# wangxb29/PPST

Measured on AMD Instinct MI355X. Metric: 512x512 portrait swaps/sec/GPU, higher is better.
Workload: dtype bf16x3 (fp32 split into hi+lo bf16, 3 MFMA passes, fp32 accumulate); 1 GPU; simple_swapping 512x512 batch=8 per GPU, generator+encoders forward only (BASELINE configs[1]); image_parallel=1 batch per rank, no data-path collective

## Files before the change

ppst_amd/csrc/conv1x1.hip:

```cpp
#include "common.h"

struct C1Args {
  const float* x;
  const unsigned char* wpack;
  const int4* steps;
  float* y;
  const float* bias;
  const float* noise;
  const float* prelu;
  float* stats;
  const float* residual;
  float noise_weight, out_scale;
  int B, hw, in_ld, out_ld, cout, nsteps, act, res_ld, n_tiles, tiles;
  int in_h, in_w, out_h, out_w, tiles_x, pad_mode;
  const float* in_ss;
  const float* in_prelu;
  int in_c, in_act;
  const float* in_res;
  int in_res_ld;
};

#define C1_GROUP 8
#define C1_BLOB 8192

typedef _Float16 __attribute__((ext_vector_type(8))) c1_half8;
template <int PREC>
__device__ __forceinline__ void c1_cvt(float v, unsigned short& h, unsigned short& l) {
  if (PREC == 0) split_bf16(v, h, l);
  else if (PREC == 3) { h = __builtin_bit_cast(unsigned short, (_Float16)v); l = 0; }
  else { h = f2bf(v); l = 0; }
}
template <int PREC>
__device__ __forceinline__ void c1_cvt8(const float (&v)[8], bf16x8& hi, bf16x8& lo) {
  if (PREC == 3) {
#pragma unroll
    for (int j = 0; j < 8; ++j) {
      unsigned short h, l;
      c1_cvt<PREC>(v[j], h, l);
      hi[j] = (short)h;
      lo[j] = (short)l;
    }
    return;
  }
  uint2 h0, l0 = make_uint2(0u, 0u), h1, l1 = make_uint2(0u, 0u);
  if (PREC == 0) {
    split_bf16x4(make_float4(v[0], v[1], v[2], v[3]), h0, l0);
    split_bf16x4(make_float4(v[4], v[5], v[6], v[7]), h1, l1);
  } else {
    h0 = f2bf_x4(make_float4(v[0], v[1], v[2], v[3]));
    h1 = f2bf_x4(make_float4(v[4], v[5], v[6], v[7]));
  }
  hi = __builtin_bit_cast(bf16x8, make_uint4(h0.x, h0.y, h1.x, h1.y));
  lo = __builtin_bit_cast(bf16x8, make_uint4(l0.x, l0.y, l1.x, l1.y));
}
template <int IOS>
__device__ __forceinline__ void c1_unpack8(float4 r, float (&v)[8]) {
  const float4 a = st_unpack4<IOS>(make_uint2(__float_as_uint(r.x), __float_as_uint(r.y)));
  const float4 b = st_unpack4<IOS>(make_uint2(__float_as_uint(r.z), __float_as_uint(r.w)));
  v[0] = a.x; v[1] = a.y; v[2] = a.z; v[3] = a.w; v[4] = b.x; v[5] = b.y; v[6] = b.z; v[7] = b.w;
}
template <int PREC>
__device__ __forceinline__ f32x4 c1_mfma(bf16x8 bh, bf16x8 bl, bf16x8 xh, bf16x8 xl, f32x4 acc) {
  if (PREC == 0) {
    acc = __builtin_amdgcn_mfma_f32_16x16x32_bf16(bh, xl, acc, 0, 0, 0);
    acc = __builtin_amdgcn_mfma_f32_16x16x32_bf16(bl, xh, acc, 0, 0, 0);
    return __builtin_amdgcn_mfma_f32_16x16x32_bf16(bh, xh, acc, 0, 0, 0);
  }
  if (PREC == 3) return __builtin_amdgcn_mfma_f32_16x16x32_f16(__builtin_bit_cast(c1_half8, bh), __builtin_bit_cast(c1_half8, xh), acc, 0, 0, 0);
  return __builtin_amdgcn_mfma_f32_16x16x32_bf16(bh, xh, acc, 0, 0, 0);
}

__device__ __forceinline__ int c1_pad(int i, int n, int mode) {
  if (mode == PPST_PAD_REFLECT) {
    if (i < 0) i = -i;
    if (i >= n) i = 2 * (n - 1) - i;
  }
  return i < 0 ? 0 : (i >= n ? n - 1 : i);
}

template <int MT, int NT, bool TAPS, bool SPEC = true, int IOS = PPST_ST_F32>
__device__ __forceinline__ void c1_epilogue(const C1Args& a, f32x4 (&acc)[MT][NT], float (&red)[8][NT > 4 ? 128 : 64][2], int b, int mblk,
                                            int ntile, int pbase, int oy0, int ox, int tid, int wave, int r16, int g) {
  const int act = a.act & 0xff;
  const bool res_after = (a.act >> 8) & 1;
  const float slope = (act == PPST_ACT_PRELU && a.prelu) ? a.prelu[0] : 0.f;
  float4 s1[NT], s2[NT];
#pragma unroll
  for (int nt = 0; nt < NT; ++nt) { s1[nt] = make_float4(0.f, 0.f, 0.f, 0.f); s2[nt] = s1[nt]; }
  const int64_t img = (int64_t)b * (TAPS ? a.out_h * a.out_w : a.hw);
  constexpr int ES = IOS == PPST_ST_F32 ? 4 : 2;
  unsigned char* const yb = (unsigned char*)a.y + img * a.out_ld * ES;
  const float* const nzb = a.noise ? a.noise + img : nullptr;
  const unsigned char* const rb = a.residual ? (const unsigned char*)a.residual + img * a.res_ld * ES : nullptr;
  const int nbase = ntile * (NT > 4 ? 128 : 64) + g * 4;
  float nzv[MT];
  float4 bva[NT];
  const __amdgpu_buffer_rsrc_t nrs = __builtin_amdgcn_make_buffer_rsrc((void*)(nzb ? (const void*)nzb : (const void*)yb), 0,
                                                                       nzb ? (TAPS ? a.out_h * a.out_w : a.hw) * 4 : 0, 0x00020000);
#pragma unroll
  for (int mt = 0; mt < MT; ++mt) {
    const int p = pbase + mt * 16 + r16;
    const bool ok = TAPS ? (oy0 + mt < a.out_h && ox < a.out_w) : p < a.hw;
    nzv[mt] = a.noise_weight * __builtin_bit_cast(float, __builtin_amdgcn_raw_buffer_load_b32(
                                   nrs, ok ? (TAPS ? (oy0 + mt) * a.out_w + ox : p) * 4 : (int)0x80000000, 0, 0));
  }
#pragma unroll
  for (int nt = 0; nt < NT; ++nt)
    bva[nt] = __builtin_bit_cast(float4, __builtin_amdgcn_raw_buffer_load_b128(__builtin_amdgcn_make_buffer_rsrc((void*)(a.bias ? (const void*)a.bias : (const void*)a.y), 0, a.bias ? a.cout * 4 : 0, 0x00020000), (nbase + nt * 16) * 4, 0, 0));
  auto epi_passes = [&](auto act_c, auto res_c) {
#pragma clang fp contract(off)
    const int ACT = act_c.value, RES = res_c.value;
#pragma unroll
  for (int mt = 0; mt < MT; ++mt) {
    const int p = pbase + mt * 16 + r16;
    if (TAPS ? (oy0 + mt >= a.out_h || ox >= a.out_w) : p >= a.hw) continue;
    const int pin = TAPS ? (oy0 + mt) * a.out_w + ox : p;
    const int yo = pin * a.out_ld, ro = pin * a.res_ld;
    const float nz = nzv[mt];
#pragma unroll
    for (int nt = 0; nt < NT; ++nt) {
      const int n0 = nbase + nt * 16;
      if (n0 >= a.cout) continue;
      float4 rv = make_float4(0.f, 0.f, 0.f, 0.f);
      const float4 bv = bva[nt];
      if (RES) rv = st_ld4<IOS>(rb, ro + n0);
      float o[4] = {acc[mt][nt][0] + bv.x + nz, acc[mt][nt][1] + bv.y + nz, acc[mt][nt][2] + bv.z + nz, acc[mt][nt][3] + bv.w + nz};
      const float r4[4] = {rv.x, rv.y, rv.z, rv.w};
#pragma unroll
      for (int c = 0; c < 4; ++c) {
        float t = o[c];
        if (RES == 1) t += r4[c];
        if (ACT == PPST_ACT_LRELU) t = (t > 0.f ? t : t * 0.2f) * 1.41421356237309515f;
        else if (ACT == PPST_ACT_PRELU) t = t >= 0.f ? t : t * slope;
        if (RES == 2) t += r4[c];
        o[c] = t * a.out_scale;
      }
      st_st4<IOS>(yb, yo + n0, make_float4(o[0], o[1], o[2], o[3]));
      s1[nt].x += o[0]; s1[nt].y += o[1]; s1[nt].z += o[2]; s1[nt].w += o[3];
      s2[nt].x += o[0] * o[0]; s2[nt].y += o[1] * o[1]; s2[nt].z += o[2] * o[2]; s2[nt].w += o[3] * o[3];
    }
  }
  };
  {
    const int resm = a.residual ? (res_after ? 2 : 1) : 0;
#define EPI_GO(A_)                                                                                    \
  do {                                                                                                \
    if (resm == 0) epi_passes(EpiC<A_>{}, EpiC<0>{});                                                 \
    else if (resm == 1) epi_passes(EpiC<A_>{}, EpiC<1>{});                                            \
    else epi_passes(EpiC<A_>{}, EpiC<2>{});                                                           \
  } while (0)
    if (!SPEC) epi_passes(EpiR{act}, EpiR{resm});
    else if (act == PPST_ACT_LRELU) EPI_GO(PPST_ACT_LRELU);
    else if (act == PPST_ACT_PRELU) EPI_GO(PPST_ACT_PRELU);
    else EPI_GO(PPST_ACT_NONE);
#undef EPI_GO
  }
  if (a.stats) {
#pragma unroll
    for (int nt = 0; nt < NT; ++nt) {
      float4 u = s1[nt], w = s2[nt];
      float* uv[8] = {&u.x, &u.y, &u.z, &u.w, &w.x, &w.y, &w.z, &w.w};
#pragma unroll
      for (int q = 0; q < 8; ++q) {
        float t = *uv[q];
        t += __builtin_bit_cast(float, __builtin_amdgcn_mov_dpp(__builtin_bit_cast(int, t), 0xB1, 0xf, 0xf, true));
        t += __builtin_bit_cast(float, __builtin_amdgcn_mov_dpp(__builtin_bit_cast(int, t), 0x4E, 0xf, 0xf, true));
        t += __builtin_bit_cast(float, __builtin_amdgcn_mov_dpp(__builtin_bit_cast(int, t), 0x141, 0xf, 0xf, true));
        t += __builtin_bit_cast(float, __builtin_amdgcn_mov_dpp(__builtin_bit_cast(int, t), 0x140, 0xf, 0xf, true));
        *uv[q] = t;
      }
      if (r16 == 0) {
        float* r = &red[wave][nt * 16 + g * 4][0];
        r[0] = u.x; r[1] = w.x; r[2] = u.y; r[3] = w.y; r[4] = u.z; r[5] = w.z; r[6] = u.w; r[7] = w.w;
      }
    }
    __syncthreads();
    if (tid < (NT > 4 ? 128 : 64)) {
      const int n = ntile * (NT > 4 ? 128 : 64) + tid;
      if (n < a.cout) {
        float t0 = 0.f, t1 = 0.f;
#pragma unroll
        for (int wv = 0; wv < 8; ++wv) { t0 += red[wv][tid][0]; t1 += red[wv][tid][1]; }
        float* o = a.stats + (((int64_t)b * a.tiles + mblk) * a.cout + n) * 2;
        o[0] = t0;
        o[1] = t1;
      }
    }
  }
}

template <int INSS, bool TAPS = false, int NT_ = 4, int PREC = 0, int IOS = PPST_ST_F32>
__global__ __launch_bounds__(512, 4) void conv1x1_stream_kernel(C1Args a) {
  constexpr int MT = 2, NT = NT_;
  constexpr bool X3 = PREC == 0;
  static_assert(IOS == PPST_ST_F32 || IOS == (PREC == 3 ? PPST_ST_F16 : PREC == 1 ? PPST_ST_BF16 : -1), "half storage: single-pass modes");
  constexpr int ES = IOS == PPST_ST_F32 ? 4 : 2;
  constexpr int BLOB1 = X3 ? C1_BLOB : C1_BLOB / 2;
  __shared__ uint4 sB[C1_GROUP * BLOB1 / 16];
  __shared__ float red[8][64][2];

  const int nwg = gridDim.x;
  int wid;
  {
    int id = blockIdx.x, q = nwg >> 3, r = nwg & 7, xcd = id & 7;
    wid = (xcd < r ? xcd * (q + 1) : r * (q + 1) + (xcd - r) * q) + (id >> 3);
  }
  const int ntile = wid % a.n_tiles;
  int mblk = wid / a.n_tiles;
  const int b = mblk / a.tiles;
  mblk -= b * a.tiles;
  const int tid = threadIdx.x, lane = tid & 63, wave = __builtin_amdgcn_readfirstlane(tid >> 6);
  const int r16 = lane & 15, g = lane >> 4;
  const int pbase = mblk * 256 + wave * 32;
  const int tyi = TAPS ? mblk / a.tiles_x : 0, txi = TAPS ? mblk - tyi * a.tiles_x : 0;
  const int oy0 = tyi * 16 + wave * 2, ox = txi * 16 + r16;
  const unsigned char* xb = (const unsigned char*)a.x + (int64_t)b * (TAPS ? a.in_h * a.in_w : a.hw) * a.in_ld * ES;
  const unsigned char* wblob = a.wpack + (int64_t)ntile * a.nsteps * BLOB1;
#if defined(__HIP_DEVICE_COMPILE__)
  typedef const __attribute__((address_space(4))) int4* StepPtr;
#else
  typedef const int4* StepPtr;
#endif
  StepPtr steps = (StepPtr)a.steps;

  int64_t aoff[MT];
  bool pok[MT];
#pragma unroll
  for (int mt = 0; mt < MT; ++mt) {
    const int p = pbase + mt * 16 + r16;
    pok[mt] = TAPS ? true : p < a.hw;
    aoff[mt] = TAPS ? 0 : (int64_t)(pok[mt] ? p : 0) * a.in_ld + g * 8;
  }
  const float in_slope = (INSS && a.in_act == PPST_ACT_PRELU && a.in_prelu) ? a.in_prelu[0] : 0.f;
  auto in_act = [&](float t) -> float {
    if (a.in_act == PPST_ACT_LRELU) return (t > 0.f ? t : t * 0.2f) * 1.41421356237309515f;
    if (a.in_act == PPST_ACT_PRELU) return t >= 0.f ? t : t * in_slope;
    return t;
  };

  f32x4 acc[MT][NT];
#pragma unroll
  for (int i = 0; i < MT; ++i)
#pragma unroll
    for (int j = 0; j < NT; ++j) acc[i][j] = (f32x4){0.f, 0.f, 0.f, 0.f};

  float4 raw[MT][2], ss[4];
  float4 rres[INSS == 2 ? MT : 1][2];
  auto a_load = [&](int4 d) {
    const int chan = d.x;
    if (TAPS) {
      int ix = ox + d.z;
      bool xok = ix >= 0 && ix < a.in_w;
      ix = c1_pad(ix, a.in_w, a.pad_mode);
#pragma unroll
      for (int mt = 0; mt < MT; ++mt) {
        int iy = oy0 + mt + d.y;
        const bool yok = iy >= 0 && iy < a.in_h;
        iy = c1_pad(iy, a.in_h, a.pad_mode);
        pok[mt] = a.pad_mode != PPST_PAD_ZERO || (xok && yok);
        aoff[mt] = ((int64_t)iy * a.in_w + ix) * a.in_ld + g * 8;
      }
    }
#pragma unroll
    for (int mt = 0; mt < MT; ++mt) {
      const float4* p = (const float4*)(xb + (aoff[mt] + chan) * ES);
      raw[mt][0] = p[0];
      if (IOS == PPST_ST_F32) raw[mt][1] = p[1];
      if (INSS == 2) {
        const int pp = pbase + mt * 16 + r16;
        const float4* q = (const float4*)(a.in_res + ((int64_t)b * a.hw + (pok[mt] ? pp : 0)) * a.in_res_ld + g * 8 + chan);
        rres[mt][0] = q[0];
        rres[mt][1] = q[1];
      }
    }
    if (INSS) {
      const float4* q = (const float4*)(a.in_ss + ((int64_t)b * a.in_c + chan + g * 8) * 2);
      ss[0] = q[0]; ss[1] = q[1]; ss[2] = q[2]; ss[3] = q[3];
    }
  };
  a_load(steps[0]);

  for (int s0 = 0; s0 < a.nsteps; s0 += C1_GROUP) {
    const int ng = a.nsteps - s0 < C1_GROUP ? a.nsteps - s0 : C1_GROUP;
    if (s0) __syncthreads();
    for (int i = tid; i < ng * (BLOB1 / 16); i += 512) sB[i] = ((const uint4*)(wblob + (int64_t)s0 * BLOB1))[i];
    __syncthreads();
    for (int sl = 0; sl < ng; ++sl) {
      const int s = s0 + sl;
      bf16x8 ah[MT], al[MT];
      bool vok[MT];
#pragma unroll
      for (int mt = 0; mt < MT; ++mt) vok[mt] = pok[mt];
#pragma unroll
      for (int mt = 0; mt < MT; ++mt) {
        if (IOS != PPST_ST_F32 && !INSS) {
          const float4 z = vok[mt] ? raw[mt][0] : make_float4(0.f, 0.f, 0.f, 0.f);
          ah[mt] = __builtin_bit_cast(bf16x8, z);
          al[mt] = ah[mt];
          continue;
        }
        float v[8] = {raw[mt][0].x, raw[mt][0].y, raw[mt][0].z, raw[mt][0].w, raw[mt][1].x, raw[mt][1].y, raw[mt][1].z, raw[mt][1].w};
        if (IOS != PPST_ST_F32) c1_unpack8<IOS>(raw[mt][0], v);
        if (INSS) {
          const float sc[8] = {ss[0].x, ss[0].z, ss[1].x, ss[1].z, ss[2].x, ss[2].z, ss[3].x, ss[3].z};
          const float sh[8] = {ss[0].y, ss[0].w, ss[1].y, ss[1].w, ss[2].y, ss[2].w, ss[3].y, ss[3].w};
#pragma unroll
          for (int j = 0; j < 8; ++j) {
            float t = sc[j] * v[j] + sh[j];
            if (INSS == 2) {
              const float4 r4 = rres[mt][j >> 2];
              t += (j & 3) == 0 ? r4.x : (j & 3) == 1 ? r4.y : (j & 3) == 2 ? r4.z : r4.w;
            }
            v[j] = in_act(t);
          }
        }
#pragma unroll
        for (int j = 0; j < 8; ++j)
          if (!vok[mt]) v[j] = 0.f;
        c1_cvt8<PREC>(v, ah[mt], al[mt]);
      }
      if (s + 1 < a.nsteps) a_load(steps[s + 1]);
      const unsigned char* bs = (const unsigned char*)sB + sl * BLOB1 + g * 1024 + r16 * 16;
#pragma unroll
      for (int nt = 0; nt < NT; ++nt) {
        const bf16x8 bh = *(const bf16x8*)(bs + nt * 256);
        bf16x8 bl = bh;
        if (X3) bl = *(const bf16x8*)(bs + nt * 256 + 4096);
#pragma unroll
        for (int mt = 0; mt < MT; ++mt) acc[mt][nt] = c1_mfma<PREC>(bh, bl, ah[mt], al[mt], acc[mt][nt]);
      }
    }
  }

  c1_epilogue<MT, NT, TAPS, X3, IOS>(a, acc, red, b, mblk, ntile, pbase, oy0, ox, tid, wave, r16, g);
}

#define C3_GROUP 9
template <int CTRL>
__device__ __forceinline__ bf16x8 c3_shift(bf16x8 edge, bf16x8 centre) {
  typedef int __attribute__((ext_vector_type(4))) i4;
  const i4 e = __builtin_bit_cast(i4, edge), c = __builtin_bit_cast(i4, centre);
  i4 r;
#pragma unroll
  for (int i = 0; i < 4; ++i) r[i] = __builtin_amdgcn_update_dpp(e[i], c[i], CTRL, 0xf, 0xf, false);
  return __builtin_bit_cast(bf16x8, r);
}

template <bool INSS, int NT_, int PREC = 0, int IOS = PPST_ST_F32>
__global__ __launch_bounds__(512, NT_ > 4 ? 2 : 4) void conv3x3_direct_kernel(C1Args a) {
  constexpr int MT = 2, NT = NT_;
  constexpr bool X3 = PREC == 0;
  static_assert(IOS == PPST_ST_F32 || IOS == (PREC == 3 ? PPST_ST_F16 : PREC == 1 ? PPST_ST_BF16 : -1), "half storage: single-pass modes");
  constexpr int ES = IOS == PPST_ST_F32 ? 4 : 2;
  constexpr int PSTR = (NT > 4 ? 128 : 64) * 16;
  constexpr int BLOB = (X3 ? 8 : 4) * PSTR;
  __shared__ uint4 sB[C3_GROUP * BLOB / 16];
  __shared__ float red[8][NT > 4 ? 128 : 64][2];
  const int tid = threadIdx.x, lane = tid & 63, wave = __builtin_amdgcn_readfirstlane(tid >> 6);
  const int r16 = lane & 15, g = lane >> 4;
  const int total = a.B * a.tiles * a.n_tiles;
  const int per = (total + (int)gridDim.x - 1) / (int)gridDim.x;
  const int w_beg = blockIdx.x * per, w_end = w_beg + per < total ? w_beg + per : total;
  const int nchunks = a.nsteps / 9;
  const bool keep_b = nchunks == 1 && a.n_tiles == 1;
  for (int wid = w_beg; wid < w_end; ++wid) {
  const int ntile = wid % a.n_tiles;
  int mblk = wid / a.n_tiles;
  const int b = mblk / a.tiles;
  mblk -= b * a.tiles;
  const int tyi = mblk / a.tiles_x, txi = mblk - tyi * a.tiles_x;
  const int oy0 = tyi * 16 + wave * 2, ox = txi * 16 + r16;
  const unsigned char* xb = (const unsigned char*)a.x + (int64_t)b * a.in_h * a.in_w * a.in_ld * ES;
  const unsigned char* wblob = a.wpack + (int64_t)ntile * a.nsteps * BLOB;
  if (wid > w_beg) __syncthreads();
#if defined(__HIP_DEVICE_COMPILE__)
  typedef const __attribute__((address_space(4))) int4* StepPtr;
#else
  typedef const int4* StepPtr;
#endif
  StepPtr steps = (StepPtr)a.steps;
  const float in_slope = (INSS && a.in_act == PPST_ACT_PRELU && a.in_prelu) ? a.in_prelu[0] : 0.f;
  auto in_act = [&](float t) -> float {
    if (a.in_act == PPST_ACT_LRELU) return (t > 0.f ? t : t * 0.2f) * 1.41421356237309515f;
    if (a.in_act == PPST_ACT_PRELU) return t >= 0.f ? t : t * in_slope;
    return t;
  };
  const int xe_raw = r16 == 0 ? ox - 1 : (r16 == 15 ? ox + 1 : ox);
  const bool cx_ok = ox < a.in_w, ex_ok = xe_raw >= 0 && xe_raw < a.in_w;
  const int cx = c1_pad(ox, a.in_w, a.pad_mode), ex = c1_pad(xe_raw, a.in_w, a.pad_mode);

  f32x4 acc[MT][NT];
#pragma unroll
  for (int i = 0; i < MT; ++i)
#pragma unroll
    for (int j = 0; j < NT; ++j) acc[i][j] = (f32x4){0.f, 0.f, 0.f, 0.f};

  float4 rawc[2], rawe[2], ss[4];
  bool okc = false, oke = false;
  auto row_load = [&](int chan, int r) {
    int iy = oy0 - 1 + r;
    const bool yok = iy >= 0 && iy < a.in_h;
    iy = c1_pad(iy, a.in_h, a.pad_mode);
    okc = a.pad_mode != PPST_PAD_ZERO || (yok && cx_ok);
    oke = a.pad_mode != PPST_PAD_ZERO || (yok && ex_ok);
    const float4* pc = (const float4*)(xb + (((int64_t)iy * a.in_w + cx) * a.in_ld + chan + g * 8) * ES);
    const float4* pe = (const float4*)(xb + (((int64_t)iy * a.in_w + ex) * a.in_ld + chan + g * 8) * ES);
    rawc[0] = pc[0];
    rawe[0] = pe[0];
    if (IOS == PPST_ST_F32) { rawc[1] = pc[1]; rawe[1] = pe[1]; }
  };
  auto ss_load = [&](int chan) {
    if (INSS) {
      const float4* q = (const float4*)(a.in_ss + ((int64_t)b * a.in_c + chan + g * 8) * 2);
      ss[0] = q[0]; ss[1] = q[1]; ss[2] = q[2]; ss[3] = q[3];
    }
  };
  auto convert = [&](const float4 (&raw)[2], bool ok, bf16x8& hi, bf16x8& lo) {
    if (IOS != PPST_ST_F32 && !INSS) {
      hi = __builtin_bit_cast(bf16x8, ok ? raw[0] : make_float4(0.f, 0.f, 0.f, 0.f));
      lo = hi;
      return;
    }
    float v[8] = {raw[0].x, raw[0].y, raw[0].z, raw[0].w, raw[1].x, raw[1].y, raw[1].z, raw[1].w};
    if (IOS != PPST_ST_F32) c1_unpack8<IOS>(raw[0], v);
    if (INSS) {
      const float sc[8] = {ss[0].x, ss[0].z, ss[1].x, ss[1].z, ss[2].x, ss[2].z, ss[3].x, ss[3].z};
      const float sh[8] = {ss[0].y, ss[0].w, ss[1].y, ss[1].w, ss[2].y, ss[2].w, ss[3].y, ss[3].w};
#pragma unroll
      for (int j = 0; j < 8; ++j) v[j] = in_act(sc[j] * v[j] + sh[j]);
    }
#pragma unroll
    for (int j = 0; j < 8; ++j)
      if (!ok) v[j] = 0.f;
    c1_cvt8<PREC>(v, hi, lo);
  };

  int chan = steps[0].x;
  ss_load(chan);
  row_load(chan, 0);
  for (int c = 0; c < nchunks; ++c) {
    if (!keep_b || wid == w_beg) {
      if (c) __syncthreads();
      for (int i = tid; i < C3_GROUP * (BLOB / 16); i += 512) sB[i] = ((const uint4*)(wblob + (int64_t)c * C3_GROUP * BLOB))[i];
      __syncthreads();
    }
    const int chan_next = c + 1 < nchunks ? steps[(c + 1) * 9].x : chan;
#pragma unroll
    for (int r = 0; r < 4; ++r) {
      bf16x8 ch, cl, eh, el;
      convert(rawc, okc, ch, cl);
      convert(rawe, oke, eh, el);
      if (r < 3) row_load(chan, r + 1);
      else if (c + 1 < nchunks) { ss_load(chan_next); row_load(chan_next, 0); }
#pragma unroll
      for (int dxi = 0; dxi < 3; ++dxi) {
        const bf16x8 fh = dxi == 0 ? c3_shift<0x111>(eh, ch) : (dxi == 1 ? ch : c3_shift<0x101>(eh, ch));
        const bf16x8 fl = dxi == 0 ? c3_shift<0x111>(el, cl) : (dxi == 1 ? cl : c3_shift<0x101>(el, cl));
#pragma unroll
        for (int mt = 0; mt < MT; ++mt) {
          const int dyi = r - mt;
          if (dyi < 0 || dyi > 2) continue;
          const unsigned char* bs = (const unsigned char*)sB + (dyi * 3 + dxi) * BLOB + g * PSTR + r16 * 16;
#pragma unroll
          for (int nt = 0; nt < NT; ++nt) {
            const bf16x8 bh = *(const bf16x8*)(bs + nt * 256);
            bf16x8 bl = bh;
            if (X3) bl = *(const bf16x8*)(bs + nt * 256 + 4 * PSTR);
            acc[mt][nt] = c1_mfma<PREC>(bh, bl, fh, fl, acc[mt][nt]);
          }
        }
        __builtin_amdgcn_sched_barrier(0);
      }
    }
    chan = chan_next;
  }
  c1_epilogue<MT, NT, true, (X3 && NT <= 4), IOS>(a, acc, red, b, mblk, ntile, 0, oy0, ox, tid, wave, r16, g);
  }
}

static inline int64_t blocks_of(const ppst_conv_args* a, int tiles, int n_tiles) { return (int64_t)a->B * tiles * n_tiles; }
int ppst_conv1x1_stream_launch(const ppst_conv_args* a, int n_tiles, int tiles, hipStream_t st) {
  C1Args k;
  k.x = (const float*)a->x; k.wpack = (const unsigned char*)a->wpack; k.steps = (const int4*)a->steps; k.y = (float*)a->y;
  k.bias = (const float*)a->bias; k.noise = (const float*)a->noise; k.prelu = (const float*)a->prelu;
  k.stats = (float*)a->stats; k.residual = (const float*)a->residual;
  k.noise_weight = a->noise_weight; k.out_scale = a->out_scale;
  k.B = a->B; k.hw = a->out_h * a->out_w; k.in_ld = a->in_ld; k.out_ld = a->out_ld; k.cout = a->cout; k.nsteps = a->nsteps;
  k.act = a->act; k.res_ld = a->res_ld; k.n_tiles = n_tiles; k.tiles = tiles;
  k.in_ss = (const float*)a->in_scale_shift; k.in_prelu = (const float*)a->in_prelu; k.in_c = a->in_c; k.in_act = a->in_act;
  k.in_res = (const float*)a->in_res; k.in_res_ld = a->in_res_ld;
  if ((int64_t)tiles * 256 < k.hw) return PPST_EINVAL;
  if (k.in_res) {
    PPST_LAUNCH((conv1x1_stream_kernel<2, false, 4, 0, PPST_ST_F32>), dim3((unsigned)blocks_of(a, tiles, n_tiles)), dim3(512), 0, st, k);
    return PPST_LAUNCH_CHECK();
  }
  const int64_t blocks = (int64_t)a->B * tiles * n_tiles;
  if (blocks > 0x7fffffff) return PPST_EINVAL;
#define LS(PREC_, IOS_)                                                                                               \
  do {                                                                                                                \
    if (k.in_ss) PPST_LAUNCH((conv1x1_stream_kernel<1, false, 4, PREC_, IOS_>), dim3((unsigned)blocks), dim3(512), 0, st, k);   \
    else PPST_LAUNCH((conv1x1_stream_kernel<0, false, 4, PREC_, IOS_>), dim3((unsigned)blocks), dim3(512), 0, st, k);          \
  } while (0)
  if (a->precision == 1) { if (a->io_st) LS(1, PPST_ST_BF16); else LS(1, PPST_ST_F32); }
  else if (a->precision == 3) { if (a->io_st) LS(3, PPST_ST_F16); else LS(3, PPST_ST_F32); }
  else LS(0, PPST_ST_F32);
#undef LS
  return PPST_LAUNCH_CHECK();
}

int ppst_conv_direct_launch(const ppst_conv_args* a, int n_tiles, int tiles_y, int tiles_x, hipStream_t st) {
  C1Args k;
  k.x = (const float*)a->x; k.wpack = (const unsigned char*)a->wpack; k.steps = (const int4*)a->steps; k.y = (float*)a->y;
  k.bias = (const float*)a->bias; k.noise = (const float*)a->noise; k.prelu = (const float*)a->prelu;
  k.stats = (float*)a->stats; k.residual = (const float*)a->residual;
  k.noise_weight = a->noise_weight; k.out_scale = a->out_scale;
  k.B = a->B; k.hw = a->out_h * a->out_w; k.in_ld = a->in_ld; k.out_ld = a->out_ld; k.cout = a->cout; k.nsteps = a->nsteps;
  k.act = a->act; k.res_ld = a->res_ld; k.n_tiles = n_tiles; k.tiles = tiles_y * tiles_x;
  k.in_ss = (const float*)a->in_scale_shift; k.in_prelu = (const float*)a->in_prelu; k.in_c = a->in_c; k.in_act = a->in_act;
  k.in_h = a->in_h; k.in_w = a->in_w; k.out_h = a->out_h; k.out_w = a->out_w; k.tiles_x = tiles_x; k.pad_mode = a->pad_mode;
  const int64_t blocks = (int64_t)a->B * k.tiles * n_tiles;
  if (blocks > 0x7fffffff) return PPST_EINVAL;
  const bool nt2 = a->cout <= 32;
#define LD(INSS_, PREC_, IOS_)                                                                                       \
  do {                                                                                                               \
    if (nt2) PPST_LAUNCH((conv1x1_stream_kernel<INSS_, true, 2, PREC_, IOS_>), dim3((unsigned)blocks), dim3(512), 0, st, k);       \
    else PPST_LAUNCH((conv1x1_stream_kernel<INSS_, true, 4, PREC_, IOS_>), dim3((unsigned)blocks), dim3(512), 0, st, k);           \
  } while (0)
#define LDP(PREC_, IOS_) do { if (k.in_ss) LD(1, PREC_, IOS_); else LD(0, PREC_, IOS_); } while (0)
  if (a->precision == 1) { if (a->io_st) LDP(1, PPST_ST_BF16); else LDP(1, PPST_ST_F32); }
  else if (a->precision == 3) { if (a->io_st) LDP(3, PPST_ST_F16); else LDP(3, PPST_ST_F32); }
  else LDP(0, PPST_ST_F32);
#undef LDP
#undef LD
  return PPST_LAUNCH_CHECK();
}

int ppst_conv3x3_direct_launch(const ppst_conv_args* a, int n_tiles, int tiles_y, int tiles_x, hipStream_t st) {
  if (a->nsteps % 9) return PPST_EINVAL;
  C1Args k;
  k.x = (const float*)a->x; k.wpack = (const unsigned char*)a->wpack; k.steps = (const int4*)a->steps; k.y = (float*)a->y;
  k.bias = (const float*)a->bias; k.noise = (const float*)a->noise; k.prelu = (const float*)a->prelu;
  k.stats = (float*)a->stats; k.residual = (const float*)a->residual;
  k.noise_weight = a->noise_weight; k.out_scale = a->out_scale;
  k.B = a->B; k.hw = a->out_h * a->out_w; k.in_ld = a->in_ld; k.out_ld = a->out_ld; k.cout = a->cout; k.nsteps = a->nsteps;
  k.act = a->act; k.res_ld = a->res_ld; k.n_tiles = n_tiles; k.tiles = tiles_y * tiles_x;
  k.in_ss = (const float*)a->in_scale_shift; k.in_prelu = (const float*)a->in_prelu; k.in_c = a->in_c; k.in_act = a->in_act;
  k.in_h = a->in_h; k.in_w = a->in_w; k.out_h = a->out_h; k.out_w = a->out_w; k.tiles_x = tiles_x; k.pad_mode = a->pad_mode;
  int64_t blocks = (int64_t)a->B * k.tiles * n_tiles;
  if (blocks > 0x7fffffff) return PPST_EINVAL;
  if (a->nsteps == 9 && n_tiles == 1 && blocks > 512) blocks = 512;
  const bool nt2 = a->cout <= 32, nt8 = a->bn == 128;
#define LD3(INSS_, PREC_, IOS_)                                                                                      \
  do {                                                                                                               \
    if (nt8 && PREC_ == 0) PPST_LAUNCH((conv3x3_direct_kernel<INSS_, 8, 0>), dim3((unsigned)blocks), dim3(512), 0, st, k);   \
    else if (nt8) return PPST_EUNSUPPORTED;                                                                          \
    else if (nt2) PPST_LAUNCH((conv3x3_direct_kernel<INSS_, 2, PREC_, IOS_>), dim3((unsigned)blocks), dim3(512), 0, st, k); \
    else PPST_LAUNCH((conv3x3_direct_kernel<INSS_, 4, PREC_, IOS_>), dim3((unsigned)blocks), dim3(512), 0, st, k);          \
  } while (0)
#define LD3P(PREC_, IOS_) do { if (k.in_ss) LD3(true, PREC_, IOS_); else LD3(false, PREC_, IOS_); } while (0)
  if (a->precision == 1) { if (a->io_st) LD3P(1, PPST_ST_BF16); else LD3P(1, PPST_ST_F32); }
  else if (a->precision == 3) { if (a->io_st) LD3P(3, PPST_ST_F16); else LD3P(3, PPST_ST_F32); }
  else LD3P(0, PPST_ST_F32);
#undef LD3P
#undef LD3
  return PPST_LAUNCH_CHECK();
}
```

Before: 158.6 swaps/s (all GPUs).

## Add 4-row-per-wave 3x3 direct conv variant with 256 threads

Adds a conv3x3 direct kernel body in which each wave computes four output rows (MT=4) instead of two. The block drops to 256 threads, and the six loaded input rows are reused across the three vertical taps. This cuts the redundant halo row loads and conversions per output row, and each weight LDS read now feeds more MFMAs. The epilogue is split into two passes to bound register pressure, with stats written per pass into a shared reduction array. In exchange it uses more registers per thread and gets lower occupancy (launch bounds 2), and it rejects very large images.

```diff
diff --git a/ppst_amd/csrc/conv1x1.hip b/ppst_amd/csrc/conv1x1.hip
--- a/ppst_amd/csrc/conv1x1.hip
+++ b/ppst_amd/csrc/conv1x1.hip
@@ -78,15 +78,14 @@
   return i < 0 ? 0 : (i >= n ? n - 1 : i);
 }
 
-template <int MT, int NT, bool TAPS, bool SPEC = true, int IOS = PPST_ST_F32>
+template <int MT, int NT, bool TAPS, bool SPEC = true, int IOS = PPST_ST_F32, int PAIRS = 1>
 __device__ __forceinline__ void c1_epilogue(const C1Args& a, f32x4 (&acc)[MT][NT], float (&red)[8][NT > 4 ? 128 : 64][2], int b, int mblk,
                                             int ntile, int pbase, int oy0, int ox, int tid, int wave, int r16, int g) {
   const int act = a.act & 0xff;
   const bool res_after = (a.act >> 8) & 1;
   const float slope = (act == PPST_ACT_PRELU && a.prelu) ? a.prelu[0] : 0.f;
+  constexpr int RP = MT / PAIRS;
   float4 s1[NT], s2[NT];
-#pragma unroll
-  for (int nt = 0; nt < NT; ++nt) { s1[nt] = make_float4(0.f, 0.f, 0.f, 0.f); s2[nt] = s1[nt]; }
   const int64_t img = (int64_t)b * (TAPS ? a.out_h * a.out_w : a.hw);
   constexpr int ES = IOS == PPST_ST_F32 ? 4 : 2;
   unsigned char* const yb = (unsigned char*)a.y + img * a.out_ld * ES;
@@ -107,11 +106,12 @@
 #pragma unroll
   for (int nt = 0; nt < NT; ++nt)
     bva[nt] = __builtin_bit_cast(float4, __builtin_amdgcn_raw_buffer_load_b128(__builtin_amdgcn_make_buffer_rsrc((void*)(a.bias ? (const void*)a.bias : (const void*)a.y), 0, a.bias ? a.cout * 4 : 0, 0x00020000), (nbase + nt * 16) * 4, 0, 0));
-  auto epi_passes = [&](auto act_c, auto res_c) {
+  auto epi_passes = [&](auto act_c, auto res_c, int mt0) {
 #pragma clang fp contract(off)
     const int ACT = act_c.value, RES = res_c.value;
 #pragma unroll
-  for (int mt = 0; mt < MT; ++mt) {
+  for (int m = 0; m < RP; ++m) {
+    const int mt = mt0 + m;
     const int p = pbase + mt * 16 + r16;
     if (TAPS ? (oy0 + mt >= a.out_h || ox >= a.out_w) : p >= a.hw) continue;
     const int pin = TAPS ? (oy0 + mt) * a.out_w + ox : p;
@@ -141,21 +141,23 @@
     }
   }
   };
-  {
+#pragma unroll
+  for (int pr = 0; pr < PAIRS; ++pr) {
+#pragma unroll
+    for (int nt = 0; nt < NT; ++nt) { s1[nt] = make_float4(0.f, 0.f, 0.f, 0.f); s2[nt] = s1[nt]; }
     const int resm = a.residual ? (res_after ? 2 : 1) : 0;
 #define EPI_GO(A_)                                                                                    \
   do {                                                                                                \
-    if (resm == 0) epi_passes(EpiC<A_>{}, EpiC<0>{});                                                 \
-    else if (resm == 1) epi_passes(EpiC<A_>{}, EpiC<1>{});                                            \
-    else epi_passes(EpiC<A_>{}, EpiC<2>{});                                                           \
+    if (resm == 0) epi_passes(EpiC<A_>{}, EpiC<0>{}, pr * RP);                                        \
+    else if (resm == 1) epi_passes(EpiC<A_>{}, EpiC<1>{}, pr * RP);                                   \
+    else epi_passes(EpiC<A_>{}, EpiC<2>{}, pr * RP);                                                  \
   } while (0)
-    if (!SPEC) epi_passes(EpiR{act}, EpiR{resm});
+    if (!SPEC) epi_passes(EpiR{act}, EpiR{resm}, pr * RP);
     else if (act == PPST_ACT_LRELU) EPI_GO(PPST_ACT_LRELU);
     else if (act == PPST_ACT_PRELU) EPI_GO(PPST_ACT_PRELU);
     else EPI_GO(PPST_ACT_NONE);
 #undef EPI_GO
-  }
-  if (a.stats) {
+    if (!a.stats) continue;
 #pragma unroll
     for (int nt = 0; nt < NT; ++nt) {
       float4 u = s1[nt], w = s2[nt];
@@ -170,10 +172,12 @@
         *uv[q] = t;
       }
       if (r16 == 0) {
-        float* r = &red[wave][nt * 16 + g * 4][0];
+        float* r = &red[wave * PAIRS + pr][nt * 16 + g * 4][0];
         r[0] = u.x; r[1] = w.x; r[2] = u.y; r[3] = w.y; r[4] = u.z; r[5] = w.z; r[6] = u.w; r[7] = w.w;
       }
     }
+  }
+  if (a.stats) {
     __syncthreads();
     if (tid < (NT > 4 ? 128 : 64)) {
       const int n = ntile * (NT > 4 ? 128 : 64) + tid;
@@ -346,8 +350,8 @@
   return __builtin_bit_cast(bf16x8, r);
 }
 
-template <bool INSS, int NT_, int PREC = 0, int IOS = PPST_ST_F32>
-__global__ __launch_bounds__(512, NT_ > 4 ? 2 : 4) void conv3x3_direct_kernel(C1Args a) {
+template <bool INSS, int NT_, int PREC, int IOS>
+__device__ __forceinline__ void c3_rows2_body(const C1Args& a) {
   constexpr int MT = 2, NT = NT_;
   constexpr bool X3 = PREC == 0;
   static_assert(IOS == PPST_ST_F32 || IOS == (PREC == 3 ? PPST_ST_F16 : PREC == 1 ? PPST_ST_BF16 : -1), "half storage: single-pass modes");
@@ -478,6 +482,191 @@
   }
 }
 
+template <bool INSS, int NT_, int PREC, int IOS>
+__device__ __forceinline__ void c3_rows4_body(const C1Args& a) {
+  constexpr int MT = 4, NT = NT_;
+  constexpr bool X3 = PREC == 0;
+  constexpr int ES = IOS == PPST_ST_F32 ? 4 : 2;
+  constexpr int PSTR = 64 * 16;
+  constexpr int BLOB = (X3 ? 8 : 4) * PSTR;
+  __shared__ uint4 sB[C3_GROUP * BLOB / 16];
+  __shared__ float red[8][64][2];
+  __shared__ float4 sS[INSS ? 16 : 1];
+  const int tid = threadIdx.x, lane = tid & 63, wave = __builtin_amdgcn_readfirstlane(tid >> 6);
+  const int r16 = lane & 15, g = lane >> 4;
+  const int total = a.B * a.tiles * a.n_tiles;
+  const int per = (total + (int)gridDim.x - 1) / (int)gridDim.x;
+  const int w_beg = blockIdx.x * per, w_end = w_beg + per < total ? w_beg + per : total;
+  const int nchunks = a.nsteps / 9;
+  const bool keep_b = nchunks == 1 && a.n_tiles == 1;
+  const unsigned char* const bs0 = (const unsigned char*)sB + g * PSTR + r16 * 16;
+  for (int wid = w_beg; wid < w_end; ++wid) {
+  const int ntile = __builtin_amdgcn_readfirstlane(wid % a.n_tiles);
+  int mblk = wid / a.n_tiles;
+  const int b = __builtin_amdgcn_readfirstlane(mblk / a.tiles);
+  mblk = __builtin_amdgcn_readfirstlane(mblk - b * a.tiles);
+  const int tyi = mblk / a.tiles_x, txi = mblk - tyi * a.tiles_x;
+  const int oy0 = tyi * 16 + wave * 4, ox = txi * 16 + r16;
+  const __amdgpu_buffer_rsrc_t xrs = __builtin_amdgcn_make_buffer_rsrc(
+      (void*)((const unsigned char*)a.x + (int64_t)b * a.in_h * a.in_w * a.in_ld * ES), 0, a.in_h * a.in_w * a.in_ld * ES, 0x00020000);
+  const unsigned char* wblob = a.wpack + (int64_t)ntile * a.nsteps * BLOB;
+  if (wid > w_beg) __syncthreads();
+#if defined(__HIP_DEVICE_COMPILE__)
+  typedef const __attribute__((address_space(4))) int4* StepPtr;
+#else
+  typedef const int4* StepPtr;
+#endif
+  StepPtr steps = (StepPtr)a.steps;
+  const float in_slope = (INSS && a.in_act == PPST_ACT_PRELU && a.in_prelu) ? a.in_prelu[0] : 0.f;
+  auto in_act = [&](float t) -> float {
+    if (a.in_act == PPST_ACT_LRELU) return (t > 0.f ? t : t * 0.2f) * 1.41421356237309515f;
+    if (a.in_act == PPST_ACT_PRELU) return t >= 0.f ? t : t * in_slope;
+    return t;
+  };
+  const int xe_raw = r16 == 0 ? ox - 1 : (r16 == 15 ? ox + 1 : ox);
+  const bool cx_ok = ox < a.in_w, ex_ok = xe_raw >= 0 && xe_raw < a.in_w;
+  const int cvo = (c1_pad(ox, a.in_w, a.pad_mode) * a.in_ld + g * 8) * ES, evo = (c1_pad(xe_raw, a.in_w, a.pad_mode) * a.in_ld + g * 8) * ES;
+
+  f32x4 acc[MT][NT];
+#pragma unroll
+  for (int i = 0; i < MT; ++i)
+#pragma unroll
+    for (int j = 0; j < NT; ++j) acc[i][j] = (f32x4){0.f, 0.f, 0.f, 0.f};
+
+  float4 rawc[4][2], rawe[4][2], ss[4];
+  bool okc[4], oke[4];
+  auto row_load = [&](int sl, int chan, int r) {
+    int iy = oy0 - 1 + r;
+    const bool yok = iy >= 0 && iy < a.in_h;
+    iy = c1_pad(iy, a.in_h, a.pad_mode);
+    okc[sl] = a.pad_mode != PPST_PAD_ZERO || (yok && cx_ok);
+    oke[sl] = a.pad_mode != PPST_PAD_ZERO || (yok && ex_ok);
+    const int so = (iy * a.in_w * a.in_ld + chan) * ES;
+    rawc[sl][0] = __builtin_bit_cast(float4, __builtin_amdgcn_raw_buffer_load_b128(xrs, cvo, so, 0));
+    rawe[sl][0] = __builtin_bit_cast(float4, __builtin_amdgcn_raw_buffer_load_b128(xrs, evo, so, 0));
+    if (IOS == PPST_ST_F32) {
+      rawc[sl][1] = __builtin_bit_cast(float4, __builtin_amdgcn_raw_buffer_load_b128(xrs, cvo + 16, so, 0));
+      rawe[sl][1] = __builtin_bit_cast(float4, __builtin_amdgcn_raw_buffer_load_b128(xrs, evo + 16, so, 0));
+    }
+  };
+  auto ss_load = [&]() {
+    if (INSS) { ss[0] = sS[g * 4]; ss[1] = sS[g * 4 + 1]; ss[2] = sS[g * 4 + 2]; ss[3] = sS[g * 4 + 3]; }
+  };
+  auto convert = [&](const float4 (&raw)[2], bool ok, bf16x8& hi, bf16x8& lo) {
+    if (IOS != PPST_ST_F32 && !INSS) {
+      hi = __builtin_bit_cast(bf16x8, ok ? raw[0] : make_float4(0.f, 0.f, 0.f, 0.f));
+      lo = hi;
+      return;
+    }
+    float v[8] = {raw[0].x, raw[0].y, raw[0].z, raw[0].w, raw[1].x, raw[1].y, raw[1].z, raw[1].w};
+    if (IOS != PPST_ST_F32) c1_unpack8<IOS>(raw[0], v);
+    if (INSS) {
+      const float sc[8] = {ss[0].x, ss[0].z, ss[1].x, ss[1].z, ss[2].x, ss[2].z, ss[3].x, ss[3].z};
+      const float sh[8] = {ss[0].y, ss[0].w, ss[1].y, ss[1].w, ss[2].y, ss[2].w, ss[3].y, ss[3].w};
+#pragma unroll
+      for (int j = 0; j < 8; ++j) v[j] = in_act(sc[j] * v[j] + sh[j]);
+    }
+#pragma unroll
+    for (int j = 0; j < 8; ++j)
+      if (!ok) v[j] = 0.f;
+    c1_cvt8<PREC>(v, hi, lo);
+  };
+  auto w_read = [&](int k, bf16x8& h, bf16x8& l) {
+    const unsigned char* bs = bs0 + (k / NT) * BLOB + (k % NT) * 256;
+    h = *(const bf16x8*)bs;
+    l = h;
+    if (X3) l = *(const bf16x8*)(bs + 4 * PSTR);
+  };
+
+  int chan = steps[0].x;
+  row_load(0, chan, 0);
+  for (int c = 0; c < nchunks; ++c) {
+#pragma unroll
+    for (int r = 1; r < 4; ++r) row_load(r, chan, r);
+    const bool fill = !keep_b || wid == w_beg;
+    if (fill) {
+      const uint4* src = (const uint4*)(wblob + (int64_t)c * C3_GROUP * BLOB) + tid;
+      const uint4 t0 = src[0], t1 = src[256], t2 = src[512], t3 = src[768], t4 = src[1024], t5 = src[1280], t6 = src[1536], t7 = src[1792], t8 = src[2048];
+      if (c) __syncthreads();
+      uint4* dst = sB + tid;
+      dst[0] = t0; dst[256] = t1; dst[512] = t2; dst[768] = t3; dst[1024] = t4; dst[1280] = t5; dst[1536] = t6; dst[1792] = t7; dst[2048] = t8;
+      if (X3) {
+        const uint4 u0 = src[2304], u1 = src[2560], u2 = src[2816], u3 = src[3072], u4 = src[3328], u5 = src[3584], u6 = src[3840], u7 = src[4096], u8 = src[4352];
+        dst[2304] = u0; dst[2560] = u1; dst[2816] = u2; dst[3072] = u3; dst[3328] = u4; dst[3584] = u5; dst[3840] = u6; dst[4096] = u7; dst[4352] = u8;
+      }
+      static_assert(C3_GROUP * (BLOB / 16) == (X3 ? 18 : 9) * 256, "weight copy: 9 or 18 vectors per thread");
+    }
+    if (INSS && tid < 16) sS[tid] = ((const float4*)(a.in_ss + ((int64_t)b * a.in_c + chan) * 2))[tid];
+    if (fill || INSS) __syncthreads();
+    const bool more = c + 1 < nchunks;
+    const int chan_next = more ? steps[(c + 1) * 9].x : chan;
+    bf16x8 wh[2], wl[2];
+    w_read(0, wh[0], wl[0]);
+    bf16x8 ch[6], cl[6], eh[6], el[6];
+#pragma unroll
+    for (int r = 0; r < 4; ++r) {
+      ss_load();
+      convert(rawc[r], okc[r], ch[r], cl[r]);
+      convert(rawe[r], oke[r], eh[r], el[r]);
+      if (r == 0) row_load(0, chan, 4);
+    }
+#pragma unroll
+    for (int dyi = 0; dyi < 3; ++dyi) {
+      if (dyi) {
+        const int r = 3 + dyi;
+        ss_load();
+        convert(rawc[0], okc[0], ch[r], cl[r]);
+        convert(rawe[0], oke[0], eh[r], el[r]);
+        if (dyi == 1) row_load(0, chan, 5);
+        else if (more) row_load(0, chan_next, 0);
+      }
+#pragma unroll
+      for (int dxi = 0; dxi < 3; ++dxi) {
+        bf16x8 fh[MT], fl[MT];
+#pragma unroll
+        for (int mt = 0; mt < MT; ++mt) {
+          const int r = mt + dyi;
+          fh[mt] = dxi == 0 ? c3_shift<0x111>(eh[r], ch[r]) : (dxi == 1 ? ch[r] : c3_shift<0x101>(eh[r], ch[r]));
+          fl[mt] = dxi == 0 ? c3_shift<0x111>(el[r], cl[r]) : (dxi == 1 ? cl[r] : c3_shift<0x101>(el[r], cl[r]));
+        }
+#pragma unroll
+        for (int nt = 0; nt < NT; ++nt) {
+          const int k = (dyi * 3 + dxi) * NT + nt;
+          if (k + 1 < 9 * NT) w_read(k + 1, wh[(k + 1) & 1], wl[(k + 1) & 1]);
+          __builtin_amdgcn_sched_barrier(0);
+          const bf16x8 bh = wh[k & 1], bl = wl[k & 1];
+          if (X3) {
+#pragma unroll
+            for (int mt = 0; mt < MT; ++mt) acc[mt][nt] = __builtin_amdgcn_mfma_f32_16x16x32_bf16(bh, fl[mt], acc[mt][nt], 0, 0, 0);
+#pragma unroll
+            for (int mt = 0; mt < MT; ++mt) acc[mt][nt] = __builtin_amdgcn_mfma_f32_16x16x32_bf16(bl, fh[mt], acc[mt][nt], 0, 0, 0);
+#pragma unroll
+            for (int mt = 0; mt < MT; ++mt) acc[mt][nt] = __builtin_amdgcn_mfma_f32_16x16x32_bf16(bh, fh[mt], acc[mt][nt], 0, 0, 0);
+          } else {
+#pragma unroll
+            for (int mt = 0; mt < MT; ++mt) acc[mt][nt] = c1_mfma<PREC>(bh, bl, fh[mt], fl[mt], acc[mt][nt]);
+          }
+          __builtin_amdgcn_sched_barrier(0);
+        }
+      }
+    }
+    chan = chan_next;
+  }
+  c1_epilogue<MT, NT, true, X3, IOS, 2>(a, acc, red, b, mblk, ntile, 0, oy0, ox, tid, wave, r16, g);
+  }
+}
+
+template <bool INSS, int NT_, int PREC, int IOS>
+constexpr bool c3_rows4() { return NT_ == 4 && !INSS && (PREC == 0 || (PREC == 3 && IOS == PPST_ST_F16)); }
+template <bool INSS, int NT_, int PREC, int IOS>
+constexpr int c3_threads() { return c3_rows4<INSS, NT_, PREC, IOS>() ? 256 : 512; }
+template <bool INSS, int NT_, int PREC = 0, int IOS = PPST_ST_F32>
+__global__ __launch_bounds__((c3_threads<INSS, NT_, PREC, IOS>()), (c3_rows4<INSS, NT_, PREC, IOS>() || NT_ > 4 ? 2 : 4)) void conv3x3_direct_kernel(C1Args a) {
+  static_assert(IOS == PPST_ST_F32 || IOS == (PREC == 3 ? PPST_ST_F16 : PREC == 1 ? PPST_ST_BF16 : -1), "half storage: single-pass modes");
+  if constexpr (c3_rows4<INSS, NT_, PREC, IOS>()) c3_rows4_body<INSS, NT_, PREC, IOS>(a);
+  else c3_rows2_body<INSS, NT_, PREC, IOS>(a);
+}
+
 static inline int64_t blocks_of(const ppst_conv_args* a, int tiles, int n_tiles) { return (int64_t)a->B * tiles * n_tiles; }
 int ppst_conv1x1_stream_launch(const ppst_conv_args* a, int n_tiles, int tiles, hipStream_t st) {
   C1Args k;
@@ -548,6 +737,7 @@
   k.in_h = a->in_h; k.in_w = a->in_w; k.out_h = a->out_h; k.out_w = a->out_w; k.tiles_x = tiles_x; k.pad_mode = a->pad_mode;
   int64_t blocks = (int64_t)a->B * k.tiles * n_tiles;
   if (blocks > 0x7fffffff) return PPST_EINVAL;
+  const bool big_image = (int64_t)a->in_h * a->in_w * a->in_ld * 4 > 0x7fffffff;
   if (a->nsteps == 9 && n_tiles == 1 && blocks > 512) blocks = 512;
   const bool nt2 = a->cout <= 32, nt8 = a->bn == 128;
 #define LD3(INSS_, PREC_, IOS_)                                                                                      \
@@ -555,7 +745,8 @@
     if (nt8 && PREC_ == 0) PPST_LAUNCH((conv3x3_direct_kernel<INSS_, 8, 0>), dim3((unsigned)blocks), dim3(512), 0, st, k);   \
     else if (nt8) return PPST_EUNSUPPORTED;                                                                          \
     else if (nt2) PPST_LAUNCH((conv3x3_direct_kernel<INSS_, 2, PREC_, IOS_>), dim3((unsigned)blocks), dim3(512), 0, st, k); \
-    else PPST_LAUNCH((conv3x3_direct_kernel<INSS_, 4, PREC_, IOS_>), dim3((unsigned)blocks), dim3(512), 0, st, k);          \
+    else if (c3_rows4<INSS_, 4, PREC_, IOS_>() && big_image) return PPST_EINVAL;                                     \
+    else PPST_LAUNCH((conv3x3_direct_kernel<INSS_, 4, PREC_, IOS_>), dim3((unsigned)blocks), dim3((c3_threads<INSS_, 4, PREC_, IOS_>())), 0, st, k); \
   } while (0)
 #define LD3P(PREC_, IOS_) do { if (k.in_ss) LD3(true, PREC_, IOS_); else LD3(false, PREC_, IOS_); } while (0)
   if (a->precision == 1) { if (a->io_st) LD3P(1, PPST_ST_BF16); else LD3P(1, PPST_ST_F32); }
```

New measurement: 159.5 swaps/s (all GPUs), median of 6. Within noise of the previous version (+0.6%).
